# wenbowen123/iros20-6d-pose-tracking

Measured on NVIDIA H100. Metric: rgbd_pair_frames_per_sec, higher is better.
Workload: dtype bf16x3 (bf16 hi/lo split operands, 3 products/MAC, fp32 accumulate)

## Files before the change

iros20-6d-pose-tracking_b200/csrc/aux_kernels.cu:

```cuda
#include "aux_kernels.h"
#include "conv_common.h"
#include "bbox.cuh"
#include "launch.h"
#include "ptx.cuh"
#include "storage.cuh"
#include <cfloat>

namespace se3tn {


__device__ __forceinline__ float norm_f32(float x, float m, float s) { return __fdiv_rn(__fsub_rn(x, m), s); }
__device__ __forceinline__ float norm_f64(float x, double m, double s) { return static_cast<float>(__ddiv_rn(__dsub_rn(static_cast<double>(x), m), s)); }

__device__ __forceinline__ float depth_offset(unsigned d, double z1000, bool gl) {
    if (d <= 100u || d >= 2000u) return 2000.f;
    return static_cast<float>(gl ? __dadd_rn(static_cast<double>(d), z1000) : __dsub_rn(static_cast<double>(d), z1000));
}

constexpr int kPreRowsMax = 88;
constexpr int kDepthLo = 101, kDepthN = 1899;

template <int THREADS>
__global__ void __launch_bounds__(THREADS, THREADS == 256 ? 4 : 1)
preprocess_kernel(PreprocessArgs a, int rows_per_cta)
// ... 728 lines not shown
    if ((threadIdx.x & 31) == 0) atomicMax(amax_bits + blockIdx.y, __float_as_uint(m));
}
cudaError_t launch_amax_bf16x3(const AmaxArgs& a, unsigned* amax_bits, cudaStream_t s) {
    if (a.n_tensors <= 0 || a.n_tensors > AmaxArgs::kMax || a.n <= 0) return cudaErrorInvalidValue;
    for (int i = 0; i < a.n_tensors; ++i) if (a.t[i].nc % 4 || a.t[i].c0 % 4) return cudaErrorInvalidValue;
    amax_bf16x3_kernel<<<dim3(132, a.n_tensors), 256, 0, s>>>(a, amax_bits);
    return cudaGetLastError();
}

__global__ void split_stack_weights_kernel(const float* __restrict__ src, uint8_t* __restrict__ dst)
{
    const int i = blockIdx.x * blockDim.x + threadIdx.x;
    if (i >= 64 * 144) return;
    const int co = i / 144, k = (i - co * 144) * 4;
    const float* w = src + co * 576 + k;
    const float v[4] = {w[0], w[1], w[2], w[3]};
    const auto x = Storage<SE3TN_PREC_BF16X3>::encode(v);
    using B = Storage<SE3TN_PREC_BF16>;
    *reinterpret_cast<uint2*>(dst + B::addr(co, 576, k)) = x.get(0);
    *reinterpret_cast<uint2*>(dst + B::addr(64 + co, 576, k)) = x.get(1);
}
__global__ void split_stem_stack_kernel(const float* __restrict__ src, uint8_t* __restrict__ dst)
{
    const int i = blockIdx.x * blockDim.x + threadIdx.x;
    if (i >= 64 * 7 * 8) return;
    const int p = i & 7, r = (i >> 3) % 7, co = i / 56;
    const float* w = src + co * 224 + r * 32 + p * 4;
    const float v[4] = {w[0], w[1], w[2], w[3]};
    const auto x = Storage<SE3TN_PREC_BF16X3>::encode(v);
    const uint2 h = x.get(0), l = x.get(1);
    *reinterpret_cast<uint4*>(dst + (static_cast<size_t>(co) * 224 + r * 32 + p * 4) * 4) = make_uint4(h.x, h.y, h.x, h.y);
    *reinterpret_cast<uint4*>(dst + (static_cast<size_t>(64 + co) * 224 + r * 32 + p * 4) * 4) = make_uint4(l.x, l.y, 0u, 0u);
}
__global__ void permute_rows64_kernel(const float* __restrict__ src, float* __restrict__ dst, int ktot)
{
    const int i = blockIdx.x * blockDim.x + threadIdx.x;
    if (i >= 64 * ktot) return;
    const int col = i / ktot, k = i - col * ktot;
    const int ch = (col & 32) | (((col >> 1) & 3) << 3) | (((col >> 3) & 3) << 1) | (col & 1);
    dst[i] = src[ch * ktot + k];
}
cudaError_t launch_permute_rows64(const float* src, float* dst, int ktot, cudaStream_t s) {
    permute_rows64_kernel<<<(64 * ktot + 255) / 256, 256, 0, s>>>(src, dst, ktot);
    return cudaGetLastError();
}
cudaError_t launch_split_stack_weights(const float* src, void* dst, bool stem, cudaStream_t s) {
    if (stem) split_stem_stack_kernel<<<(64 * 7 * 8 + 127) / 128, 128, 0, s>>>(src, static_cast<uint8_t*>(dst));
    else split_stack_weights_kernel<<<(64 * 144 + 255) / 256, 256, 0, s>>>(src, static_cast<uint8_t*>(dst));
    return cudaGetLastError();
}

__global__ void pose_update_kernel(const double* poses_in, const float* __restrict__ trans,
                                   const float* __restrict__ rot, float tn, float rn,
                                   double* poses_out , int n)
{
    ptx::grid_dep_launch();
    ptx::grid_dep_wait();
    const int i = blockIdx.x * blockDim.x + threadIdx.x;
    if (i >= n) return;
    const float tr[3] = {trans[i * 3 + 0], trans[i * 3 + 1], trans[i * 3 + 2]};
    const float ro[3] = {rot[i * 3 + 0], rot[i * 3 + 1], rot[i * 3 + 2]};
    pose_update_one(poses_in + i * 16, tr, ro, tn, rn, poses_out + i * 16);
}

cudaError_t launch_pose_update(const double* poses_in, const float* trans, const float* rot, float tn, float rn,
                               double* poses_out, int n, cudaStream_t s) {
    if (n <= 0) return cudaSuccess;
    return launch_kernel(pose_update_kernel, dim3((n + 31) / 32), dim3(32), 0, s, true, poses_in, trans, rot, tn, rn, poses_out, n);
}

__device__ __forceinline__ void inv_transpose3(const double* m, double* o) {
    const double c00 = m[4] * m[8] - m[5] * m[7], c01 = m[5] * m[6] - m[3] * m[8], c02 = m[3] * m[7] - m[4] * m[6];
    const double det = m[0] * c00 + m[1] * c01 + m[2] * c02;
    const double id = 1.0 / det;
    o[0] = c00 * id; o[1] = c01 * id; o[2] = c02 * id;
    o[3] = (m[2] * m[7] - m[1] * m[8]) * id; o[4] = (m[0] * m[8] - m[2] * m[6]) * id; o[5] = (m[1] * m[6] - m[0] * m[7]) * id;
// ... 66 lines not shown
```

iros20-6d-pose-tracking_b200/csrc/aux_kernels.h:

```cpp
#pragma once
#include <cstdint>
#include <cuda_runtime.h>

namespace se3tn {

constexpr int kImg = 176;
constexpr int kStemH = kImg + 6;
constexpr int kStemW = kImg + 8;
constexpr size_t kStemImgFloats = static_cast<size_t>(kStemH) * kStemW * 4;

struct PreprocessArgs {
    const uint8_t* frame_rgb;
    const uint16_t* frame_depth;
    int H, W;
    double fx, fy, cx, cy;
    const double* poses;
    const double* object_width;
    const uint8_t* rgbA;
    const uint16_t* depthA;
    const int* weight_ids;
    const float* mean32; const float* std32;
    const double* mean64; const double* std64;
    int stats_f64;
    int stats_rows;
// ... 21 lines not shown
cudaError_t launch_crop_seg(const uint8_t* frame_rgb, const uint16_t* frame_depth, const uint8_t* seg, int H, int W, const int* bbox,
                            const int* class_ids, int n, int out_h, int out_w, uint8_t* crop_rgb, uint16_t* crop_depth,
                            uint8_t* crop_seg, int* count, cudaStream_t s);
struct AppendArgs {
    const uint8_t* rgbA; const uint16_t* depthA; const uint8_t* rgbB; const uint16_t* depthB;
    const int* count; const double* A_in_cam; const double* B_in_cam; const int* queue_ids;
    int n, num_queues, cap, min_count;
    int* tails;
    unsigned* done;
    uint8_t* q_rgbA; uint16_t* q_depthA; uint8_t* q_rgbB; uint16_t* q_depthB; double* q_A; double* q_B;
};
cudaError_t launch_append_pairs(const AppendArgs& a, cudaStream_t s);
cudaError_t launch_nchw_to_stem(const float* src, float* dst, int n, int precision, cudaStream_t s);
cudaError_t launch_maxpool(const float* in, float* out, int n_img, int Hin, int Win, int C, cudaStream_t s);
cudaError_t launch_head_pooled(const float* part , const float* fcw, const float* fcb, float* out_trans, float* out_rot,
                               int n_img, int npix, const int* img_wid, const float* const* fc_table,
                               const double* poses_in, double* poses_out, float tn, float rn, const LossArgs& loss,
                               unsigned* zero_words, int n_zero, cudaStream_t s);
cudaError_t launch_loss_reduce(const float* sq, int n, float* sums, cudaStream_t s);
cudaError_t launch_pair_loss(const float* trans, const float* rot, const double* trans_label, const double* rot_label,
                             const LossArgs& loss, int n, float* sums, cudaStream_t s);
cudaError_t launch_head(const float* x, const float* fcw, const float* fcb, float* out_trans, float* out_rot,
                        int n_img, int npix, cudaStream_t s);
cudaError_t launch_nhwc_to_nchw(const void* in, float* out, int n_img, int HW, int C, int precision, cudaStream_t s,
                                const float* fp8_scale = nullptr);
cudaError_t launch_encode_weights(int precision, const float* src, void* dst, int rows, int ktot, cudaStream_t s);
cudaError_t launch_encode_weights_fp8(const float* src, void* dst, float* row_scale, int rows, int ktot, cudaStream_t s);
struct AmaxArgs {
    static constexpr int kMax = 8;
    struct Tensor { const uint8_t* buf; int pixels, C, c0, nc; } t[kMax];
    int n_tensors, n;
};
cudaError_t launch_amax_bf16x3(const AmaxArgs& a, unsigned* amax_bits, cudaStream_t s);
cudaError_t launch_permute_rows64(const float* src , float* dst, int ktot, cudaStream_t s);
cudaError_t launch_split_stack_weights(const float* src, void* dst , bool stem, cudaStream_t s);
cudaError_t launch_pose_update(const double* poses_in, const float* trans, const float* rot, float tn, float rn,
                               double* poses_out, int n, cudaStream_t s);
cudaError_t launch_so3_log(const double* poses_a, const double* poses_b, double tn, double rn,
                           double* trans_label, double* rot_label, int n, cudaStream_t s);

}
```

iros20-6d-pose-tracking_b200/csrc/conv_common.h:

```cpp
#pragma once
#include <cstdint>
#include <cuda.h>
#include <cuda_runtime.h>

namespace se3tn {

constexpr int kMaxTaps = 9;
constexpr int kBlockM = 128;
constexpr int kChunkBytes = 128;

enum Act : int { ACT_NONE = 0, ACT_RELU = 1, ACT_SELU = 2 };
enum { KIND_S1 = 0, KIND_S2 = 1, KIND_STEM = 2 };

struct Tap {
    int16_t dy, dx;
};

struct ConvGeom {
    int Hin, Win, in_cstride, in_coff;
    int Ho, Wo, stride;
    int cin;
    int cout;
    int groups;
    int num_taps;
    int n_img;
    Tap taps[kMaxTaps];
    int out_cstride, out_coff;
    int res_cstride, res_coff;
    int act;
};

struct ConvPtrs {
    const float* in;
    const float* w;
    const float* bias;
    const float* res;
    float* out;
};

constexpr int kLayersPerSet = 14;
constexpr int kPoolSlices = 8;

struct LayerDesc {
    CUtensorMap amap[4];
    CUtensorMap bmap;
// ... 73 lines not shown
```

iros20-6d-pose-tracking_b200/csrc/conv_wgmma.cu:

```cuda
#include "conv_common.h"
#include "launch.h"
#include "ptx.cuh"
#include "storage.cuh"
#include <algorithm>

namespace se3tn {
namespace {

constexpr int kThreads2 = 384;
constexpr int kPoolPitch = 68;
constexpr int kPoolStageBytes = 121 * kPoolPitch * 4;
constexpr int kPoolStageAlloc = (kPoolStageBytes + 1023) & ~1023;
constexpr int kWgRowBytes = 64 * kChunkBytes;

template <int KIND> struct KTab;
template <> struct KTab<KIND_S1> {
    static constexpr int NU = 3;
    static constexpr int kAUnit = 19 * 1024;
    __host__ __device__ static constexpr int ntaps(int) { return 3; }
    __host__ __device__ static constexpr int wtap(int u, int k) { return k * 3 + u; }
    __host__ __device__ static constexpr int amap(int) { return 0; }
    __host__ __device__ static constexpr int c1(int u) { return u - 1; }
    __host__ __device__ static constexpr int c2(int) { return -1; }
    __host__ __device__ static constexpr int rows(int) { return 11 * 13; }
// ... 422 lines not shown
                    float4 mx = make_float4(-3.0e38f, -3.0e38f, -3.0e38f, -3.0e38f);
#pragma unroll
                    for (int dy = 0; dy < 3; ++dy)
#pragma unroll
                        for (int dx = 0; dx < 3; ++dx) {
                            const float4 s4 = *reinterpret_cast<const float4*>(stage + ((2 * ppy + dy) * 11 + 2 * ppx + dx) * kPoolPitch + c4);
                            mx.x = fmaxf(mx.x, s4.x); mx.y = fmaxf(mx.y, s4.y); mx.z = fmaxf(mx.z, s4.z); mx.w = fmaxf(mx.w, s4.w);
                        }
                    const float v4[4] = {selu_fast(mx.x + pb4.x), selu_fast(mx.y + pb4.y), selu_fast(mx.z + pb4.z), selu_fast(mx.w + pb4.w)};
                    S::encode(v4).store(L.out + S::addr((static_cast<size_t>(n0) * L.Ho + oy) * L.Wo + ox, L.out_c, L.out_coff + c4));
                }
                if constexpr (kShareStage) stage_turn.pass();
                else if constexpr (!PP) { if (C::kPoolBufs == 1) ptx::bar_sync(kEpiBar, 256); }
            }
            if (tstamp) tile_stamp(p.tile_trace, tile, 3);
        }
        if constexpr (PP) {
            turn.end(it);
            if constexpr (kShareStage) stage_turn.end(it);
        }
        if (stamp) { trace_stamp(p.trace, 4); trace_stamp(p.trace, 6); }
    }

    __syncthreads();
    if (threadIdx.x == 0) trace_exit(p.trace);
}

template <int PREC> struct TCfg {
    static constexpr int BN = 128;
    static constexpr int kAcc = BN / 2;
    static constexpr int kAStages = 3;
    static constexpr int kBStages = 6;
    static constexpr int kBTile = BN * kChunkBytes;
    static constexpr int kEpiPitch = 36;
    static constexpr int kEpiWarpBytes = 16 * kEpiPitch * 4 + 128;
    static constexpr int kEpiBytes = 8 * kEpiWarpBytes;
    static constexpr int kSched = 4;
    static constexpr int kAUnit = KTab<KIND_S1>::kAUnit;
    static_assert(kAUnit == KTab<KIND_S2>::kAUnit, "A ring stage size");
    static constexpr int kSmem = kAStages * kAUnit + kBStages * kBTile + ((kEpiBytes + 1023) & ~1023) + 1024 + 512;
    static_assert(kSmem <= 232448, "shared memory budget");
};
constexpr int kTaps3 = 9;

struct UnitCoord { int l, img, tx, ty, n_tile, grp, c0, c1, piece, gidx; };
__device__ __forceinline__ void unit_stamp(const TrunkParams& p, int u, int k) {
    if (p.trace && u < 2048) p.trace[256 * 8 + u * 5 + k] = k == 4 ? (gtimer() & ~0xffull) | (blockIdx.x & 0xff) : gtimer();
}

__device__ __forceinline__ int unit_layer(const TrunkParams& p, int u) {
    int l = 0;
#pragma unroll
    for (int i = 1; i < kTrunkMaxLayers; ++i) if (i < p.n_layers && u >= p.layer[i].unit_base) l = i;
    return l;
}

__device__ __forceinline__ UnitCoord decode_unit(const TrunkParams& p, int u) {
    UnitCoord c;
    c.l = unit_layer(p, u);
    const LayerDesc& L = p.layer[c.l];
    int local = u - L.unit_base;
    c.piece = 0; c.c0 = 0; c.c1 = L.chunks;
    if (p.ksplit > 1) {
        c.piece = local % p.ksplit; local /= p.ksplit;
        c.c0 = c.piece * L.chunks / p.ksplit; c.c1 = (c.piece + 1) * L.chunks / p.ksplit;
    }
    c.gidx = L.base_unit0 + local;
    const int im = local / L.units_per_image;
    int r = local - im * L.units_per_image;
    c.img = p.img_first + im;
    c.n_tile = r % L.n_tiles; r /= L.n_tiles;
    c.grp = r % L.groups; r /= L.groups;
    c.ty = r / L.tiles_x; c.tx = r - c.ty * L.tiles_x;
    return c;
}

template <int KIND, int PREC>
__device__ __forceinline__ void trunk_load_weights(const LayerDesc& L, const CUtensorMap* bm, const UnitCoord& c, uint8_t* sB,
                                                   uint64_t* b_full, uint64_t* b_empty, Ring<TCfg<PREC>::kBStages>& ring)
{
    using KT = KTab<KIND>;
    using C = TCfg<PREC>;
    const int wrow = c.grp * L.cout + c.n_tile * C::BN;
    for (int ch = c.c0; ch < c.c1; ++ch) {
#pragma unroll
        for (int u = 0; u < KT::NU; ++u) {
#pragma unroll
            for (int k = 0; k < KT::ntaps(u); ++k) {
                ptx::mbar_wait(&b_empty[ring.stage], ring.producer_parity());
                ptx::mbar_arrive_expect_tx(&b_full[ring.stage], C::kBTile);
                ptx::tma_load_2d(sB + ring.stage * C::kBTile, bm, &b_full[ring.stage], KT::wtap(u, k) * L.cin_words + ch * 32, wrow);
                ring.next();
            }
        }
    }
}

template <int KIND, int PREC>
__device__ __forceinline__ void trunk_mma_unit(float (&acc)[2][TCfg<PREC>::kAcc], const Consumer& cs, const Turn& turn, int chunks,
                                               uint8_t* sA, uint8_t* sB, uint64_t* a_full, uint64_t* a_empty, uint64_t* b_full,
                                               uint64_t* b_empty, Ring<TCfg<PREC>::kAStages>& a_ring, Ring<TCfg<PREC>::kBStages>& b_ring,
                                               unsigned long long* trace, bool first_unit, unsigned long long* ustamp)
{
    using KT = KTab<KIND>;
    using C = TCfg<PREC>;
    const bool stamp = cs.leader();
    uint32_t fresh = 0;
    int pend_b = -1, pend_a = -1;
    turn.wait();
    for (int ch = 0; ch < chunks; ++ch) {
#pragma unroll
        for (int u = 0; u < KT::NU; ++u) {
            ptx::mbar_wait(&a_full[a_ring.stage], a_ring.consumer_parity());
            if (first_unit && ch == 0 && u == 0 && stamp) trace_stamp(trace, 3);
            if (ustamp && ch == 0 && u == 0 && stamp) *ustamp = gtimer();
            const uint32_t a_unit_lo = desc_lo(sA + a_ring.stage * C::kAUnit);
#pragma unroll
            for (int k = 0; k < KT::ntaps(u); ++k) {
                ptx::mbar_wait(&b_full[b_ring.stage], b_ring.consumer_parity());
                if (first_unit && ch == 0 && u == 0 && k == 0 && stamp) trace_stamp(trace, 2);
                const uint32_t b_lo = desc_lo(sB + b_ring.stage * C::kBTile);
                ptx::wgmma_fence();
#pragma unroll
                for (int hf = 0; hf < 2; ++hf) {
                    const uint32_t a_lo = a_unit_lo + hf * (kWgRowBytes >> 4) + k * kRowShift * (kChunkBytes >> 4);
                    if constexpr (PREC == SE3TN_PREC_BF16X3) {
                        constexpr int AO[6] = {0, 2, 4, 6, 0, 2};
                        constexpr int BO[6] = {0, 2, 0, 2, 4, 6};
#pragma unroll
                        for (int i = 0; i < 6; ++i)
                            ptx::wgmma_bf16_n128(acc[hf], mk_desc(a_lo + AO[i]), mk_desc(b_lo + BO[i]), fresh | (i ? 1u : 0u));
                    } else {
                        mma_chunk<PREC, C::BN>(acc[hf], a_lo, b_lo, fresh);
                    }
                }
                ptx::wgmma_commit();
                ptx::wgmma_wait<1>();
                if (cs.leader()) {
                    if (pend_b >= 0) ptx::mbar_arrive(&b_empty[pend_b]);
                    if (pend_a >= 0) ptx::mbar_arrive(&a_empty[pend_a]);
                }
                pend_b = b_ring.stage;
                pend_a = (k + 1 == KT::ntaps(u)) ? a_ring.stage : -1;
                fresh = 1u;
                b_ring.next();
            }
            a_ring.next();
        }
    }
    turn.pass();
    ptx::wgmma_wait<0>();
    ptx::wgmma_reg_fence(acc[0]);
    ptx::wgmma_reg_fence(acc[1]);
    if (cs.leader()) {
        if (pend_b >= 0) ptx::mbar_arrive(&b_empty[pend_b]);
        if (pend_a >= 0) ptx::mbar_arrive(&a_empty[pend_a]);
    }
}

template <int PREC>
__global__ void __launch_bounds__(kThreads2, 1)
conv_trunk_kernel(const __grid_constant__ TrunkParams p)
{
    using C = TCfg<PREC>;
    constexpr int BN = C::BN;
    extern __shared__ uint8_t smem_raw[];
    uint8_t* smem = reinterpret_cast<uint8_t*>((reinterpret_cast<uintptr_t>(smem_raw) + 1023) & ~uintptr_t(1023));
    uint8_t* sA = smem;
    uint8_t* sB = sA + C::kAStages * C::kAUnit;
    uint8_t* sT = sB + C::kBStages * C::kBTile;
    uint64_t* bars = reinterpret_cast<uint64_t*>(sT + ((C::kEpiBytes + 1023) & ~1023));
    uint64_t* a_full = bars;
    uint64_t* a_empty = a_full + C::kAStages;
    uint64_t* b_full = a_empty + C::kAStages;
    uint64_t* b_empty = b_full + C::kBStages;
    uint64_t* sched_full = b_empty + C::kBStages;
    uint64_t* sched_empty = sched_full + C::kSched;
    int* sched_slot = reinterpret_cast<int*>(sched_empty + C::kSched);

    ptx::grid_dep_launch();
    if (threadIdx.x == 0) trace_stamp(p.trace, 0);
    const int warp = threadIdx.x >> 5;
    const int lane = threadIdx.x & 31;
    unsigned* done = p.sched + 1;

    if (threadIdx.x == 0) {
        for (int s = 0; s < C::kAStages; ++s) { ptx::mbar_init(&a_full[s], 1); ptx::mbar_init(&a_empty[s], 1); }
        for (int s = 0; s < C::kBStages; ++s) { ptx::mbar_init(&b_full[s], 1); ptx::mbar_init(&b_empty[s], 1); }
        for (int s = 0; s < C::kSched; ++s) { ptx::mbar_init(&sched_full[s], 1); ptx::mbar_init(&sched_empty[s], 9); }
        ptx::fence_barrier_init();
        ptx::fence_proxy_async();
    }
    __syncthreads();
    if (threadIdx.x == 0) trace_stamp(p.trace, 1);

    Ring<C::kSched> sring;
    auto next_unit = [&](bool whole_warp) -> int {
        ptx::mbar_wait(&sched_full[sring.stage], sring.consumer_parity());
        int u = 0;
        if (lane == 0) u = sched_slot[sring.stage];
        if (whole_warp) u = __shfl_sync(0xffffffffu, u, 0);
        if (lane == 0) ptx::mbar_arrive(&sched_empty[sring.stage]);
        sring.next();
        return u;
// ... 24 lines not shown
                            const long long t0 = clock64();
                            while (static_cast<unsigned>(ptx::ld_acquire_gpu(flag)) < L.dep_target) {
                                __nanosleep(64);
                                if (clock64() - t0 > (1ll << 34)) ptx::timeout_trap();
                            }
                        }
                        ptx::fence_proxy_async_all();
                    }
                    unit_stamp(p, u, 0);
                    const int cbase = c.grp * L.in_gstride_words;
                    if (L.kind == KIND_S1) load_a_units<KIND_S1>(L, c.tx * 11, c.ty * 11, cbase, c.img, c.c0, c.c1, sA, a_full, a_empty, a_ring);
                    else                   load_a_units<KIND_S2>(L, c.tx * 11, c.ty * 11, cbase, c.img, c.c0, c.c1, sA, a_full, a_empty, a_ring);
                    u = dealt ? u + static_cast<int>(gridDim.x) : static_cast<int>(atomicAdd(p.sched, 1u));
                }
            }
        } else if (warp == 1) {
            if (lane == 0) {
                if (!p.img_wid) for (int l = 0; l < p.n_layers; ++l) ptx::prefetch_tmap(&p.layer[l].bmap);
                Ring<C::kBStages> b_ring;
                for (;;) {
                    const int u = next_unit(false);
                    if (u >= p.total_units) break;
                    const UnitCoord c = decode_unit(p, u);
                    const LayerDesc& L = p.layer[c.l];
                    const CUtensorMap* bm = p.img_wid ? p.gbmaps + p.img_wid[c.img] * kLayersPerSet + L.li : &L.bmap;
                    if (L.kind == KIND_S1) trunk_load_weights<KIND_S1, PREC>(L, bm, c, sB, b_full, b_empty, b_ring);
                    else                   trunk_load_weights<KIND_S2, PREC>(L, bm, c, sB, b_full, b_empty, b_ring);
                }
            }
        }
    } else {
        ptx::setmaxnreg_inc<kConsumerRegs>();
        using S = Storage<PREC>;
        using R4 = Raw<PREC, 4>;
        ptx::grid_dep_wait();
        const Consumer cs;
        const int cw = cs.cw;
        float (*stg)[C::kEpiPitch] = reinterpret_cast<float (*)[C::kEpiPitch]>(sT + cs.ew * C::kEpiWarpBytes);
        int* rowtab = reinterpret_cast<int*>(sT + cs.ew * C::kEpiWarpBytes + 16 * C::kEpiPitch * 4);
        const int grp = lane & 7, sub = lane >> 3;
        Ring<C::kAStages> a_ring;
        Ring<C::kBStages> b_ring;
        const Turn turn{kTurnBar, cs.cg};
        turn.begin();
        for (int it = 0;; ++it) {
            const int u = next_unit(true);
            const bool mine = turn.mine(it);
            if (u >= p.total_units) { turn.end(it); break; }
            const UnitCoord c = decode_unit(p, u);
            const LayerDesc& L = p.layer[c.l];
            const int chunks = L.chunks / p.ksplit;
            if (!mine) {
                a_ring.skip(chunks * (L.kind == KIND_S1 ? KTab<KIND_S1>::NU : KTab<KIND_S2>::NU));
                b_ring.skip(chunks * kTaps3);
                continue;
            }
            {
                const int rw = 64 * (lane >> 4) + 16 * cw + (lane & 15);
                const int py = rw / 11, px = rw - py * 11;
                const int y = c.ty * 11 + py, x = c.tx * 11 + px;
                const bool valid = (rw < 121) && (y < L.Ho) && (x < L.Wo);
                __syncwarp();
                rowtab[lane] = valid ? (c.img * L.Ho + y) * L.Wo + x : -1;
                __syncwarp();
            }
            const int ch0 = c.grp * L.cout + c.n_tile * BN;
            const float* bias_base = p.img_wid ? p.gbias[p.img_wid[c.img] * kLayersPerSet + L.li] : L.bias;
            float4 b4[BN / 32];
#pragma unroll
            for (int bi = 0; bi < BN / 32; ++bi) b4[bi] = __ldg(reinterpret_cast<const float4*>(bias_base + ch0 + 32 * bi + grp * 4));
            const float* q8 = nullptr;
            float s_res = 1.f, inv_out = 1.f;
            if constexpr (PREC == SE3TN_PREC_FP8) {
                q8 = p.img_wid ? p.gfp8[p.img_wid[c.img]] : p.fp8;
                const int qg = L.q_grp_ch ? ch0 / L.q_grp_ch : 0;
                if (L.q_res >= 0) s_res = __ldg(q8 + L.q_res + qg);
                if (L.q_out >= 0) inv_out = 1.f / __ldg(q8 + L.q_out + qg);
            }

            float acc[2][C::kAcc];
#pragma unroll
            for (int i = 0; i < C::kAcc; ++i) { acc[0][i] = 0.f; acc[1][i] = 0.f; }
            unsigned long long* ust = (p.trace && u < 2048) ? p.trace + 256 * 8 + u * 5 + 1 : nullptr;
            if (L.kind == KIND_S1) trunk_mma_unit<KIND_S1, PREC>(acc, cs, turn, chunks, sA, sB, a_full, a_empty, b_full, b_empty, a_ring, b_ring, p.trace, it == 0, ust);
            else                   trunk_mma_unit<KIND_S2, PREC>(acc, cs, turn, chunks, sA, sB, a_full, a_empty, b_full, b_empty, a_ring, b_ring, p.trace, it == 0, ust);
            if (cs.leader()) { unit_stamp(p, u, 2); unit_stamp(p, u, 3); if (it == 0) trace_stamp(p.trace, 5); }
            int pix[2][4];
#pragma unroll
            for (int hf = 0; hf < 2; ++hf)
#pragma unroll
                for (int k = 0; k < 4; ++k) pix[hf][k] = rowtab[16 * hf + 4 * k + sub];

            if (L.res && L.dep_layer >= 0) {
                if (lane == 0) (void)ptx::ld_acquire_gpu(reinterpret_cast<const int*>(done + L.dep_layer * p.max_batch + c.img));
                __syncwarp();
            }
            const bool split = p.ksplit > 1;
            auto slice_of = [&](int pc) -> float* {
                return p.partial + ((static_cast<size_t>(c.gidx) * p.ksplit + pc) * 4 + cw) * (32 * BN);
            };
            unsigned own = 0xFu;
            if (split) {
                float4* d4 = reinterpret_cast<float4*>(slice_of(c.piece)) + lane;
#pragma unroll
                for (int hf = 0; hf < 2; ++hf)
#pragma unroll
                    for (int q = 0; q < C::kAcc / 4; ++q)
                        d4[(hf * C::kAcc / 4 + q) * 32] = make_float4(acc[hf][4 * q], acc[hf][4 * q + 1], acc[hf][4 * q + 2], acc[hf][4 * q + 3]);
                __threadfence();
                __syncwarp();
                if (lane == 0) atomicAdd(p.slice_cnt + c.gidx * 4 + cw, 1u);
                own = 0u;
#pragma unroll
                for (int bi = 0; bi < BN / 32; ++bi)
                    if (bi * p.ksplit / (BN / 32) == c.piece) own |= 1u << bi;
                if (lane == 0) {
                    const int* cnt = reinterpret_cast<const int*>(p.slice_cnt + c.gidx * 4 + cw);
                    const long long t0 = clock64();
                    while (ptx::ld_acquire_gpu(cnt) < p.ksplit) {
                        __nanosleep(32);
                        if (clock64() - t0 > (1ll << 34)) ptx::timeout_trap();
                    }
                }
                __syncwarp();
                __threadfence();
#pragma unroll
                for (int hf = 0; hf < 2; ++hf)
#pragma unroll
                    for (int bi = 0; bi < BN / 32; ++bi) {
                        if (!((own >> bi) & 1u)) continue;
#pragma unroll
                        for (int jj = 0; jj < 4; ++jj) {
                            float4 v[kSplitK];
#pragma unroll
                            for (int pc = 0; pc < kSplitK; ++pc)
                                if (pc < p.ksplit) v[pc] = __ldcg(reinterpret_cast<const float4*>(slice_of(pc)) + lane + (hf * C::kAcc / 4 + 4 * bi + jj) * 32);
                            float4 a = make_float4(0.f, 0.f, 0.f, 0.f);
#pragma unroll
                            for (int pc = 0; pc < kSplitK; ++pc)
                                if (pc < p.ksplit) { a.x += v[pc].x; a.y += v[pc].y; a.z += v[pc].z; a.w += v[pc].w; }
                            acc[hf][16 * bi + 4 * jj] = a.x; acc[hf][16 * bi + 4 * jj + 1] = a.y; acc[hf][16 * bi + 4 * jj + 2] = a.z; acc[hf][16 * bi + 4 * jj + 3] = a.w;
                        }
                    }
            }
#pragma unroll
            for (int hf = 0; hf < 2; ++hf) {
                const int slice = 4 * hf + cw;
#pragma unroll
                for (int bi = 0; bi < BN / 32; ++bi) {
                    if (!((own >> bi) & 1u)) continue;
                    const int chan = ch0 + 32 * bi;
                    R4 rr[4];
                    if (L.res) {
#pragma unroll
                        for (int k = 0; k < 4; ++k) {
                            rr[k] = R4{};
                            if (pix[hf][k] >= 0) {
                                const uint8_t* rp = L.res + S::addr(pix[hf][k], L.res_c, chan + grp * 4);
#pragma unroll
                                for (int q = 0; q < R4::kPieces; ++q) rr[k].set(q, __ldcg(R4::at(rp, q)));
                            }
                        }
                    }
                    __syncwarp();
#pragma unroll
                    for (int jj = 0; jj < 4; ++jj)
#pragma unroll
                        for (int h = 0; h < 2; ++h)
                            *reinterpret_cast<float2*>(&stg[cs.R + 8 * h][8 * jj + 2 * cs.m]) = make_float2(acc[hf][16 * bi + 4 * jj + 2 * h], acc[hf][16 * bi + 4 * jj + 2 * h + 1]);
                    float4 m4 = make_float4(1.f, 1.f, 1.f, 1.f);
                    if constexpr (PREC == SE3TN_PREC_FP8) m4 = __ldg(reinterpret_cast<const float4*>(q8 + L.fp8_mul + chan + grp * 4));
                    __syncwarp();
                    float4 a4[4];
#pragma unroll
                    for (int k = 0; k < 4; ++k) {
                        a4[k] = *reinterpret_cast<const float4*>(&stg[4 * k + sub][grp * 4]);
                        if constexpr (PREC == SE3TN_PREC_FP8) {
                            a4[k].x = a4[k].x * m4.x + b4[bi].x; a4[k].y = a4[k].y * m4.y + b4[bi].y;
                            a4[k].z = a4[k].z * m4.z + b4[bi].z; a4[k].w = a4[k].w * m4.w + b4[bi].w;
                        } else {
                            a4[k].x += b4[bi].x; a4[k].y += b4[bi].y; a4[k].z += b4[bi].z; a4[k].w += b4[bi].w;
                        }
                    }
                    if (L.res) {
#pragma unroll
                        for (int k = 0; k < 4; ++k) {
                            float r[4];
                            S::decode(rr[k], r);
                            if constexpr (PREC == SE3TN_PREC_FP8) { r[0] *= s_res; r[1] *= s_res; r[2] *= s_res; r[3] *= s_res; }
                            a4[k].x += r[0]; a4[k].y += r[1]; a4[k].z += r[2]; a4[k].w += r[3];
                        }
                    }
                    float4 psum = make_float4(0.f, 0.f, 0.f, 0.f);
#pragma unroll
                    for (int k = 0; k < 4; ++k) {
                        float4 o = a4[k];
                        o.x = act_apply(o.x, L.act); o.y = act_apply(o.y, L.act); o.z = act_apply(o.z, L.act); o.w = act_apply(o.w, L.act);
                        if (pix[hf][k] < 0) continue;
                        if (L.pool_part) { psum.x += o.x; psum.y += o.y; psum.z += o.z; psum.w += o.w; continue; }
                        if constexpr (PREC == SE3TN_PREC_FP8) { o.x *= inv_out; o.y *= inv_out; o.z *= inv_out; o.w *= inv_out; }
                        const float o4[4] = {o.x, o.y, o.z, o.w};
                        S::encode(o4).store(L.out + S::addr(pix[hf][k], L.out_c, L.out_coff + chan + grp * 4));
                    }
                    if (L.pool_part) {
#pragma unroll
                        for (int off = 8; off <= 16; off <<= 1) {
                            psum.x += __shfl_xor_sync(0xffffffffu, psum.x, off); psum.y += __shfl_xor_sync(0xffffffffu, psum.y, off);
                            psum.z += __shfl_xor_sync(0xffffffffu, psum.z, off); psum.w += __shfl_xor_sync(0xffffffffu, psum.w, off);
                        }
                        if (sub == 0)
                            *reinterpret_cast<float4*>(L.pool_part + (static_cast<size_t>(c.img) * kPoolSlices + slice) * L.out_c + L.out_coff + chan + grp * 4) = psum;
                    }
                }
            }
            if (c.l + 1 < p.n_layers) {
                ptx::fence_proxy_async_all();
                __threadfence();
                __syncwarp();
                if (lane == 0) atomicAdd(done + c.l * p.max_batch + c.img, 1u);
            }
            if (cs.leader()) unit_stamp(p, u, 4);
        }
        if (threadIdx.x == 128) { trace_stamp(p.trace, 4); trace_stamp(p.trace, 6); }
    }

    __syncthreads();
    if (threadIdx.x == 0) trace_exit(p.trace);
}

template <int KIND, int PREC>
cudaError_t launch_resident_t(const ResidentParams& p, int num_sms, bool pdl, cudaStream_t stream) {
    using C = RCfg<KIND, resident_prec(PREC)>;
    if (PREC == SE3TN_PREC_FP8 && ((!p.fp8 && !p.gfp8) || p.L.q_out < 0)) return cudaErrorInvalidValue;
    const int tiles_per_tap = (C::kStack == 2) ? 1 : p.L.chunks;
    if ((KIND == KIND_STEM ? 7 : 9) * tiles_per_tap > C::kMaxWTiles) return cudaErrorInvalidValue;
    if (C::kStack == 2 && KIND == KIND_S1 && p.L.chunks != 2) return cudaErrorInvalidValue;
    if (p.L.cout != 64 || p.L.groups != 1 || p.L.n_tiles != 1 || p.m_tiles <= 0) return cudaErrorInvalidValue;
    const bool pp = p.m_tiles > num_sms;
    const cudaError_t e = pp ? set_max_dynamic_smem<conv_resident_kernel<KIND, PREC, true>>(C::kSmem)
                             : set_max_dynamic_smem<conv_resident_kernel<KIND, PREC, false>>(C::kSmem);
    if (e != cudaSuccess) return e;
    return launch_kernel(pp ? conv_resident_kernel<KIND, PREC, true> : conv_resident_kernel<KIND, PREC, false>,
                         dim3(std::min(p.m_tiles, num_sms)), dim3(kThreads2), C::kSmem, stream, pdl, p);
}

template <int PREC>
// ... 52 lines not shown
```

iros20-6d-pose-tracking_b200/csrc/se3tn.cu:

```cuda
#include "../../include/se3tn.h"
#include "conv_common.h"
#include "aux_kernels.h"
#include "metrics.h"
#include "overlay.h"
#include "render.h"
#include <dlfcn.h>
#include "depth_fill.h"
#include "storage.cuh"

#include <algorithm>
#include <cmath>
#include <cstdio>
#include <cstdlib>
#include <cstring>
#include <map>
#include <memory>
#include <string>
#include <type_traits>
#include <vector>

using namespace se3tn;

namespace {

// ... 572 lines not shown
}

int queue_preprocess(se3tn_ctx* c, PreprocessArgs a, int n, cudaStream_t s) {
    a.mean32 = c->d_mean32.get(); a.std32 = c->d_std32.get(); a.mean64 = c->d_mean64.get(); a.std64 = c->d_std64.get();
    a.stats_f64 = c->stats_f64; a.stats_rows = c->stats_rows;
    a.stemA = c->buf[B_X0A]; a.stemB = c->buf[B_X0B];
    { ProfScope ps(c, 17, s); CU_TRY(c, launch_preprocess(a, n, s)); }
    ++c->launches;
    return SE3TN_OK;
}

int queue_render(se3tn_ctx* c, const double* K, const double* poses, const double* object_width, const int32_t* mesh_ids, int n,
                 int mode, int H, int W, uint8_t* rgbA, uint16_t* depthA, cudaStream_t s) {
    RenderArgs a;
    a.poses = poses; a.object_width = object_width; a.mesh_ids = mesh_ids; a.meshes = c->d_meshes.get(); a.n_meshes = c->mesh_rows;
    a.fx = K[0]; a.fy = K[1]; a.cx = K[2]; a.cy = K[3];
    a.rgb = rgbA; a.depth = depthA;
    a.mode = mode == SE3TN_RENDER_PYRENDER ? 1 : 0; a.vw = W; a.vh = H;
    a.projected = c->render_proj.get(); a.uniforms = c->render_unif.get(); a.max_nv = c->render_max_nv;
    { ProfScope ps(c, 20, s); CU_TRY(c, launch_render(a, n, s)); }
    c->launches += 2;
    return SE3TN_OK;
}

int prepare_weights(se3tn_ctx* c, DeviceWeights& w, const float* blob) {
    const size_t floats = blob_floats();
    CU_TRY(c, dev_alloc(w.blob, floats));
    for (int p : kTensorPrecs) CU_TRY(c, dev_alloc(w.conv[p], floats * prec_bytes_per_channel(p)));
    CU_TRY(c, dev_alloc(w.conv[SE3TN_PREC_FP8], floats));
    CU_TRY(c, dev_alloc(w.fp8, kFp8BlockFloats));
    CU_TRY(c, dev_alloc(w.fp8_sw, kFp8WRows));
    CU_TRY(c, dev_alloc(w.stack, 8 * 128 * 288 * sizeof(float)));
    CU_TRY(c, dev_alloc(w.perm, 6 * 64 * 576));
    DevBuf<float> perm_tmp;
    CU_TRY(c, dev_alloc(perm_tmp, 64 * 576));
    CU_TRY(c, cudaDeviceSynchronize());
    CU_TRY(c, cudaMemcpy(w.blob.get(), blob, floats * sizeof(float), cudaMemcpyHostToDevice));
    size_t off = 0;
    for (int li = 0; li < 14; ++li) {
        const LayerSpec& L = kLayers[li];
        const int rows = layer_rows(L), ktot = layer_ktot(L);
        w.w_off[li] = off; off += static_cast<size_t>(rows) * ktot;
        w.b_off[li] = off; off += rows;
        const float* wsrc = w.blob.get() + w.w_off[li];
        auto conv_dst = [&](int p) { return w.conv[p].get() + w.w_off[li] * prec_bytes_per_channel(p); };
        char what[64];
        int rc = SE3TN_OK;
        if (li >= kFirstTrunkLayer) {
            snprintf(what, sizeof what, "layer %d weights", li);
            for (int p : kTensorPrecs) {
                CU_TRY(c, launch_encode_weights(p, wsrc, conv_dst(p), rows, ktot, 0));
                if (!rc) rc = make_map2(c, &w.bmap[p][li], conv_dst(p), ktot * prec_bytes_per_channel(p) / 4, rows, L.block_n, what);
            }
            int sw_off = 0;
            for (int l = 0; l < li - kFirstTrunkLayer; ++l) sw_off += kFp8TrunkRows[l];
            CU_TRY(c, launch_encode_weights_fp8(wsrc, conv_dst(SE3TN_PREC_FP8), w.fp8_sw.get() + sw_off, rows, ktot, 0));
            if (!rc) rc = make_map2(c, &w.bmap[SE3TN_PREC_FP8][li], conv_dst(SE3TN_PREC_FP8), ktot / 4, rows, L.block_n, what);
        } else {
            const bool stem = (L.kind == K_STEM);
            void* w_tf32 = conv_dst(SE3TN_PREC_TF32);
            if (!stem) {
                if (ktot != 576 || rows != 64) return fail(c, SE3TN_ERR_STATE, "resident layer shape");
                CU_TRY(c, launch_permute_rows64(wsrc, perm_tmp.get(), 576, 0));
                wsrc = perm_tmp.get(); w_tf32 = w.perm.get() + static_cast<size_t>(li - 2) * 64 * 576;
            }
            snprintf(what, sizeof what, "layer %d resident weights", li);
            CU_TRY(c, launch_encode_weights(SE3TN_PREC_TF32, wsrc, w_tf32, 64, ktot, 0));
            rc = make_map2(c, &w.bmap[SE3TN_PREC_TF32][li], w_tf32, ktot, 64, 64, what);
            uint8_t* sdst = w.stack.get() + static_cast<size_t>(li) * 128 * 288 * sizeof(float);
            CU_TRY(c, launch_split_stack_weights(wsrc, sdst, stem, 0));
            if (!rc) rc = make_map2(c, &w.bmap[SE3TN_PREC_BF16X3][li], sdst, stem ? 224 : 288, 128, 128, what);
            for (int p : {SE3TN_PREC_BF16, SE3TN_PREC_FP16}) {
                if (stem) w.bmap[p][li] = w.bmap[stem_input_prec(p)][li];
                else {
                    CU_TRY(c, launch_encode_weights(p, wsrc, conv_dst(p), 64, ktot, 0));
                    if (!rc) rc = make_map2(c, &w.bmap[p][li], conv_dst(p), 288, 64, 64, what);
                }
            }
            w.bmap[SE3TN_PREC_FP8][li] = w.bmap[resident_prec(SE3TN_PREC_FP8)][li];
        }
        if (rc) return rc;
    }
    w.fc_off = off;
    CU_TRY(c, cudaDeviceSynchronize());
    w.fp8_sw_host.resize(kFp8WRows);
    CU_TRY(c, cudaMemcpy(w.fp8_sw_host.data(), w.fp8_sw.get(), kFp8WRows * sizeof(float), cudaMemcpyDeviceToHost));
    CU_TRY(c, cudaMemset(w.fp8.get(), 0, kFp8BlockFloats * sizeof(float)));
    CU_TRY(c, cudaDeviceSynchronize());
    return SE3TN_OK;
}

int upload_fp8(se3tn_ctx* c, WeightSet& ws, const float* scales) {
    const DeviceWeights& w = *ws.dev;
    std::vector<float> blk(kFp8BlockFloats, 0.f);
    for (int i = 0; i < SE3TN_FP8_SCALES; ++i) blk[i] = scales[i];
    int sw = 0;
    for (int l = 0; l < kTrunkMaxLayers; ++l) {
        float* mul = blk.data() + fp8_mul_off(l);
        for (int co = 0; co < kFp8TrunkRows[l]; ++co)
            mul[co] = scales[kFp8In[l] + (fp8_in_grouped(l) ? co / kFp8HeadCh : 0)] * w.fp8_sw_host[sw + co];
        sw += kFp8TrunkRows[l];
    }
    CU_TRY(c, cudaDeviceSynchronize());
    CU_TRY(c, cudaMemcpy(w.fp8.get(), blk.data(), blk.size() * sizeof(float), cudaMemcpyHostToDevice));
    memcpy(ws.fp8_scales, scales, sizeof ws.fp8_scales);
    ws.has_fp8 = true;
    return SE3TN_OK;
}

bool fp16_weights_fit(const float* blob) {
    size_t off = 0;
    for (const LayerSpec& L : kLayers) {
        const size_t nw = static_cast<size_t>(layer_rows(L)) * layer_ktot(L);
        if (L.kind != K_STEM)
            for (size_t i = 0; i < nw; ++i)
                if (std::fabs(blob[off + i]) > kFp16Max) return false;
        off += nw + layer_rows(L);
    }
    return true;
// ... 1121 lines not shown
```

Measured before the change: 35990.

## Permute trunk weight rows to match MMA fragments and drop smem epilogue staging

Trunk-layer weight rows are permuted at load time so each thread's wgmma accumulator fragment holds 8 contiguous output channels. The epilogue can then apply bias, residual, activation and the store straight from registers. This removes the shared-memory staging buffer, its warp syncs and the row table, and pooled sums are reduced with shuffles instead. Residual loads are prefetched one block ahead. The risk is correctness if the row permutation and the fp8 per-row scale remapping are inconsistent, plus higher register pressure. Trace stamps are also narrowed to 32 bits.

```diff
diff --git a/iros20-6d-pose-tracking_b200/csrc/aux_kernels.cu b/iros20-6d-pose-tracking_b200/csrc/aux_kernels.cu
--- a/iros20-6d-pose-tracking_b200/csrc/aux_kernels.cu
+++ b/iros20-6d-pose-tracking_b200/csrc/aux_kernels.cu
@@ -784,16 +784,16 @@
     *reinterpret_cast<uint4*>(dst + (static_cast<size_t>(co) * 224 + r * 32 + p * 4) * 4) = make_uint4(h.x, h.y, h.x, h.y);
     *reinterpret_cast<uint4*>(dst + (static_cast<size_t>(64 + co) * 224 + r * 32 + p * 4) * 4) = make_uint4(l.x, l.y, 0u, 0u);
 }
-__global__ void permute_rows64_kernel(const float* __restrict__ src, float* __restrict__ dst, int ktot)
+__global__ void permute_rows_kernel(const float* __restrict__ src, float* __restrict__ dst, int rows, int ktot)
 {
     const int i = blockIdx.x * blockDim.x + threadIdx.x;
-    if (i >= 64 * ktot) return;
+    if (i >= rows * ktot) return;
     const int col = i / ktot, k = i - col * ktot;
-    const int ch = (col & 32) | (((col >> 1) & 3) << 3) | (((col >> 3) & 3) << 1) | (col & 1);
-    dst[i] = src[ch * ktot + k];
-}
-cudaError_t launch_permute_rows64(const float* src, float* dst, int ktot, cudaStream_t s) {
-    permute_rows64_kernel<<<(64 * ktot + 255) / 256, 256, 0, s>>>(src, dst, ktot);
+    dst[i] = src[static_cast<size_t>(fragment_row_channel(col)) * ktot + k];
+}
+cudaError_t launch_permute_rows(const float* src, float* dst, int rows, int ktot, cudaStream_t s) {
+    if (rows % 32) return cudaErrorInvalidValue;
+    permute_rows_kernel<<<(rows * ktot + 255) / 256, 256, 0, s>>>(src, dst, rows, ktot);
     return cudaGetLastError();
 }
 cudaError_t launch_split_stack_weights(const float* src, void* dst, bool stem, cudaStream_t s) {
diff --git a/iros20-6d-pose-tracking_b200/csrc/aux_kernels.h b/iros20-6d-pose-tracking_b200/csrc/aux_kernels.h
--- a/iros20-6d-pose-tracking_b200/csrc/aux_kernels.h
+++ b/iros20-6d-pose-tracking_b200/csrc/aux_kernels.h
@@ -77,7 +77,7 @@
     int n_tensors, n;
 };
 cudaError_t launch_amax_bf16x3(const AmaxArgs& a, unsigned* amax_bits, cudaStream_t s);
-cudaError_t launch_permute_rows64(const float* src , float* dst, int ktot, cudaStream_t s);
+cudaError_t launch_permute_rows(const float* src , float* dst, int rows , int ktot, cudaStream_t s);
 cudaError_t launch_split_stack_weights(const float* src, void* dst , bool stem, cudaStream_t s);
 cudaError_t launch_pose_update(const double* poses_in, const float* trans, const float* rot, float tn, float rn,
                                double* poses_out, int n, cudaStream_t s);
diff --git a/iros20-6d-pose-tracking_b200/csrc/conv_common.h b/iros20-6d-pose-tracking_b200/csrc/conv_common.h
--- a/iros20-6d-pose-tracking_b200/csrc/conv_common.h
+++ b/iros20-6d-pose-tracking_b200/csrc/conv_common.h
@@ -11,6 +11,10 @@
 
 enum Act : int { ACT_NONE = 0, ACT_RELU = 1, ACT_SELU = 2 };
 enum { KIND_S1 = 0, KIND_S2 = 1, KIND_STEM = 2 };
+
+__host__ __device__ constexpr int fragment_row_channel(int row) {
+    return (row & ~31) | (((row >> 1) & 3) << 3) | (((row >> 3) & 3) << 1) | (row & 1);
+}
 
 struct Tap {
     int16_t dy, dx;
diff --git a/iros20-6d-pose-tracking_b200/csrc/conv_wgmma.cu b/iros20-6d-pose-tracking_b200/csrc/conv_wgmma.cu
--- a/iros20-6d-pose-tracking_b200/csrc/conv_wgmma.cu
+++ b/iros20-6d-pose-tracking_b200/csrc/conv_wgmma.cu
@@ -478,20 +478,21 @@
     static constexpr int kAStages = 3;
     static constexpr int kBStages = 6;
     static constexpr int kBTile = BN * kChunkBytes;
-    static constexpr int kEpiPitch = 36;
-    static constexpr int kEpiWarpBytes = 16 * kEpiPitch * 4 + 128;
-    static constexpr int kEpiBytes = 8 * kEpiWarpBytes;
     static constexpr int kSched = 4;
     static constexpr int kAUnit = KTab<KIND_S1>::kAUnit;
     static_assert(kAUnit == KTab<KIND_S2>::kAUnit, "A ring stage size");
-    static constexpr int kSmem = kAStages * kAUnit + kBStages * kBTile + ((kEpiBytes + 1023) & ~1023) + 1024 + 512;
+    static constexpr int kSmem = kAStages * kAUnit + kBStages * kBTile + 1024 + 512;
     static_assert(kSmem <= 232448, "shared memory budget");
 };
 constexpr int kTaps3 = 9;
 
 struct UnitCoord { int l, img, tx, ty, n_tile, grp, c0, c1, piece, gidx; };
+constexpr int kTraceUnits = 5 * 256 * 8 * 2 / 5;
+__device__ __forceinline__ unsigned* unit_stamps(const TrunkParams& p, int u) {
+    return (p.trace && u < kTraceUnits) ? reinterpret_cast<unsigned*>(p.trace + 256 * 8) + u * 5 : nullptr;
+}
 __device__ __forceinline__ void unit_stamp(const TrunkParams& p, int u, int k) {
-    if (p.trace && u < 2048) p.trace[256 * 8 + u * 5 + k] = k == 4 ? (gtimer() & ~0xffull) | (blockIdx.x & 0xff) : gtimer();
+    if (unsigned* s = unit_stamps(p, u)) s[k] = k == 4 ? (static_cast<unsigned>(gtimer()) & ~0xffu) | (blockIdx.x & 0xff) : static_cast<unsigned>(gtimer());
 }
 
 __device__ __forceinline__ int unit_layer(const TrunkParams& p, int u) {
@@ -546,7 +547,7 @@
 __device__ __forceinline__ void trunk_mma_unit(float (&acc)[2][TCfg<PREC>::kAcc], const Consumer& cs, const Turn& turn, int chunks,
                                                uint8_t* sA, uint8_t* sB, uint64_t* a_full, uint64_t* a_empty, uint64_t* b_full,
                                                uint64_t* b_empty, Ring<TCfg<PREC>::kAStages>& a_ring, Ring<TCfg<PREC>::kBStages>& b_ring,
-                                               unsigned long long* trace, bool first_unit, unsigned long long* ustamp)
+                                               unsigned long long* trace, bool first_unit, unsigned* ustamp)
 {
     using KT = KTab<KIND>;
     using C = TCfg<PREC>;
@@ -559,7 +560,7 @@
         for (int u = 0; u < KT::NU; ++u) {
             ptx::mbar_wait(&a_full[a_ring.stage], a_ring.consumer_parity());
             if (first_unit && ch == 0 && u == 0 && stamp) trace_stamp(trace, 3);
-            if (ustamp && ch == 0 && u == 0 && stamp) *ustamp = gtimer();
+            if (ustamp && ch == 0 && u == 0 && stamp) *ustamp = static_cast<unsigned>(gtimer());
             const uint32_t a_unit_lo = desc_lo(sA + a_ring.stage * C::kAUnit);
 #pragma unroll
             for (int k = 0; k < KT::ntaps(u); ++k) {
@@ -614,8 +615,7 @@
     uint8_t* smem = reinterpret_cast<uint8_t*>((reinterpret_cast<uintptr_t>(smem_raw) + 1023) & ~uintptr_t(1023));
     uint8_t* sA = smem;
     uint8_t* sB = sA + C::kAStages * C::kAUnit;
-    uint8_t* sT = sB + C::kBStages * C::kBTile;
-    uint64_t* bars = reinterpret_cast<uint64_t*>(sT + ((C::kEpiBytes + 1023) & ~1023));
+    uint64_t* bars = reinterpret_cast<uint64_t*>(sB + C::kBStages * C::kBTile);
     uint64_t* a_full = bars;
     uint64_t* a_empty = a_full + C::kAStages;
     uint64_t* b_full = a_empty + C::kAStages;
@@ -706,13 +706,10 @@
     } else {
         ptx::setmaxnreg_inc<kConsumerRegs>();
         using S = Storage<PREC>;
-        using R4 = Raw<PREC, 4>;
+        using R8 = Raw<PREC, 8>;
         ptx::grid_dep_wait();
         const Consumer cs;
         const int cw = cs.cw;
-        float (*stg)[C::kEpiPitch] = reinterpret_cast<float (*)[C::kEpiPitch]>(sT + cs.ew * C::kEpiWarpBytes);
-        int* rowtab = reinterpret_cast<int*>(sT + cs.ew * C::kEpiWarpBytes + 16 * C::kEpiPitch * 4);
-        const int grp = lane & 7, sub = lane >> 3;
         Ring<C::kAStages> a_ring;
         Ring<C::kBStages> b_ring;
         const Turn turn{kTurnBar, cs.cg};
@@ -729,20 +726,8 @@
                 b_ring.skip(chunks * kTaps3);
                 continue;
             }
-            {
-                const int rw = 64 * (lane >> 4) + 16 * cw + (lane & 15);
-                const int py = rw / 11, px = rw - py * 11;
-                const int y = c.ty * 11 + py, x = c.tx * 11 + px;
-                const bool valid = (rw < 121) && (y < L.Ho) && (x < L.Wo);
-                __syncwarp();
-                rowtab[lane] = valid ? (c.img * L.Ho + y) * L.Wo + x : -1;
-                __syncwarp();
-            }
             const int ch0 = c.grp * L.cout + c.n_tile * BN;
             const float* bias_base = p.img_wid ? p.gbias[p.img_wid[c.img] * kLayersPerSet + L.li] : L.bias;
-            float4 b4[BN / 32];
-#pragma unroll
-            for (int bi = 0; bi < BN / 32; ++bi) b4[bi] = __ldg(reinterpret_cast<const float4*>(bias_base + ch0 + 32 * bi + grp * 4));
             const float* q8 = nullptr;
             float s_res = 1.f, inv_out = 1.f;
             if constexpr (PREC == SE3TN_PREC_FP8) {
@@ -755,15 +740,21 @@
             float acc[2][C::kAcc];
 #pragma unroll
             for (int i = 0; i < C::kAcc; ++i) { acc[0][i] = 0.f; acc[1][i] = 0.f; }
-            unsigned long long* ust = (p.trace && u < 2048) ? p.trace + 256 * 8 + u * 5 + 1 : nullptr;
+            unsigned* ust = unit_stamps(p, u);
+            if (ust) ++ust;
             if (L.kind == KIND_S1) trunk_mma_unit<KIND_S1, PREC>(acc, cs, turn, chunks, sA, sB, a_full, a_empty, b_full, b_empty, a_ring, b_ring, p.trace, it == 0, ust);
             else                   trunk_mma_unit<KIND_S2, PREC>(acc, cs, turn, chunks, sA, sB, a_full, a_empty, b_full, b_empty, a_ring, b_ring, p.trace, it == 0, ust);
             if (cs.leader()) { unit_stamp(p, u, 2); unit_stamp(p, u, 3); if (it == 0) trace_stamp(p.trace, 5); }
-            int pix[2][4];
+            int pix[2][2];
 #pragma unroll
             for (int hf = 0; hf < 2; ++hf)
 #pragma unroll
-                for (int k = 0; k < 4; ++k) pix[hf][k] = rowtab[16 * hf + 4 * k + sub];
+                for (int h = 0; h < 2; ++h) {
+                    const int rw = cs.row(hf, h);
+                    const int py = rw / 11, px = rw - py * 11;
+                    const int y = c.ty * 11 + py, x = c.tx * 11 + px;
+                    pix[hf][h] = (rw < 121) && (y < L.Ho) && (x < L.Wo) ? (c.img * L.Ho + y) * L.Wo + x : -1;
+                }
 
             if (L.res && L.dep_layer >= 0) {
                 if (lane == 0) (void)ptx::ld_acquire_gpu(reinterpret_cast<const int*>(done + L.dep_layer * p.max_batch + c.img));
@@ -817,75 +808,97 @@
                         }
                     }
             }
-#pragma unroll
-            for (int hf = 0; hf < 2; ++hf) {
-                const int slice = 4 * hf + cw;
-#pragma unroll
-                for (int bi = 0; bi < BN / 32; ++bi) {
-                    if (!((own >> bi) & 1u)) continue;
-                    const int chan = ch0 + 32 * bi;
-                    R4 rr[4];
+            struct BlockRes { R8 res[2]; };
+            auto load_res = [&](int hf, int bi, BlockRes& a) {
+                const int chan = ch0 + 32 * bi + 8 * cs.m;
+#pragma unroll
+                for (int h = 0; h < 2; ++h) {
+                    a.res[h] = R8{};
+                    if (L.res && pix[hf][h] >= 0) {
+                        const uint8_t* rp = L.res + S::addr(pix[hf][h], L.res_c, chan);
+#pragma unroll
+                        for (int q = 0; q < R8::kPieces; ++q) a.res[h].set(q, __ldcg(R8::at(rp, q)));
+                    }
+                }
+            };
+            constexpr int kBlocks = 2 * BN / 32;
+            BlockRes cur, nxt;
+            if (own & 1u) load_res(0, 0, cur);
+#pragma unroll
+            for (int q = 0; q < kBlocks; ++q) {
+                const int hf = q >> 2, bi = q & 3;
+                if (q + 1 < kBlocks && ((own >> ((q + 1) & 3)) & 1u)) load_res((q + 1) >> 2, (q + 1) & 3, nxt);
+                if (!((own >> bi) & 1u)) { cur = nxt; continue; }
+                const int chan = ch0 + 32 * bi + 8 * cs.m;
+                const float4 bA = __ldg(reinterpret_cast<const float4*>(bias_base + chan)), bB = __ldg(reinterpret_cast<const float4*>(bias_base + chan + 4));
+                const float bias8[8] = {bA.x, bA.y, bA.z, bA.w, bB.x, bB.y, bB.z, bB.w};
+                float mul8[8] = {1.f, 1.f, 1.f, 1.f, 1.f, 1.f, 1.f, 1.f};
+                if constexpr (PREC == SE3TN_PREC_FP8) {
+                    const float4 mA = __ldg(reinterpret_cast<const float4*>(q8 + L.fp8_mul + chan));
+                    const float4 mB = __ldg(reinterpret_cast<const float4*>(q8 + L.fp8_mul + chan + 4));
+                    mul8[0] = mA.x; mul8[1] = mA.y; mul8[2] = mA.z; mul8[3] = mA.w; mul8[4] = mB.x; mul8[5] = mB.y; mul8[6] = mB.z; mul8[7] = mB.w;
+                }
+                float o[2][8];
+#pragma unroll
+                for (int h = 0; h < 2; ++h) {
+                    float* v = o[h];
+#pragma unroll
+                    for (int jj = 0; jj < 4; ++jj)
+#pragma unroll
+                        for (int e = 0; e < 2; ++e) {
+                            const float a = acc[hf][16 * bi + 4 * jj + 2 * h + e];
+                            if constexpr (PREC == SE3TN_PREC_FP8) v[2 * jj + e] = a * mul8[2 * jj + e] + bias8[2 * jj + e];
+                            else                                  v[2 * jj + e] = a + bias8[2 * jj + e];
+                        }
                     if (L.res) {
-#pragma unroll
-                        for (int k = 0; k < 4; ++k) {
-                            rr[k] = R4{};
-                            if (pix[hf][k] >= 0) {
-                                const uint8_t* rp = L.res + S::addr(pix[hf][k], L.res_c, chan + grp * 4);
-#pragma unroll
-                                for (int q = 0; q < R4::kPieces; ++q) rr[k].set(q, __ldcg(R4::at(rp, q)));
-                            }
+                        float r[8];
+                        S::decode(cur.res[h], r);
+#pragma unroll
+                        for (int e = 0; e < 8; ++e) {
+                            if constexpr (PREC == SE3TN_PREC_FP8) r[e] *= s_res;
+                            v[e] += r[e];
                         }
                     }
-                    __syncwarp();
-#pragma unroll
-                    for (int jj = 0; jj < 4; ++jj)
-#pragma unroll
-                        for (int h = 0; h < 2; ++h)
-                            *reinterpret_cast<float2*>(&stg[cs.R + 8 * h][8 * jj + 2 * cs.m]) = make_float2(acc[hf][16 * bi + 4 * jj + 2 * h], acc[hf][16 * bi + 4 * jj + 2 * h + 1]);
-                    float4 m4 = make_float4(1.f, 1.f, 1.f, 1.f);
-                    if constexpr (PREC == SE3TN_PREC_FP8) m4 = __ldg(reinterpret_cast<const float4*>(q8 + L.fp8_mul + chan + grp * 4));
-                    __syncwarp();
-                    float4 a4[4];
-#pragma unroll
-                    for (int k = 0; k < 4; ++k) {
-                        a4[k] = *reinterpret_cast<const float4*>(&stg[4 * k + sub][grp * 4]);
-                        if constexpr (PREC == SE3TN_PREC_FP8) {
-                            a4[k].x = a4[k].x * m4.x + b4[bi].x; a4[k].y = a4[k].y * m4.y + b4[bi].y;
-                            a4[k].z = a4[k].z * m4.z + b4[bi].z; a4[k].w = a4[k].w * m4.w + b4[bi].w;
-                        } else {
-                            a4[k].x += b4[bi].x; a4[k].y += b4[bi].y; a4[k].z += b4[bi].z; a4[k].w += b4[bi].w;
+                    if (L.act == ACT_SELU) {
+#pragma unroll
+                        for (int e = 0; e < 8; ++e) v[e] = selu_fast(v[e]);
+                    } else if (L.act == ACT_RELU) {
+#pragma unroll
+                        for (int e = 0; e < 8; ++e) v[e] = fmaxf(v[e], 0.f);
+                    }
+                    if (L.pool_part || pix[hf][h] < 0) continue;
+                    if constexpr (PREC == SE3TN_PREC_FP8) {
+#pragma unroll
+                        for (int e = 0; e < 8; ++e) v[e] *= inv_out;
+                    }
+                    S::encode(o[h]).store(L.out + S::addr(pix[hf][h], L.out_c, L.out_coff + chan));
+                }
+                if (L.pool_part) {
+                    const bool lo = cs.R < 4;
+                    float s[4];
+#pragma unroll
+                    for (int e = 0; e < 4; ++e) {
+                        float own_v[2], other[2];
+#pragma unroll
+                        for (int h = 0; h < 2; ++h) {
+                            const float mine = pix[hf][h] >= 0 ? (lo ? o[h][e] : o[h][4 + e]) : 0.f;
+                            const float give = pix[hf][h] >= 0 ? (lo ? o[h][4 + e] : o[h][e]) : 0.f;
+                            own_v[h] = mine;
+                            other[h] = __shfl_xor_sync(0xffffffffu, give, 16);
                         }
-                    }
-                    if (L.res) {
-#pragma unroll
-                        for (int k = 0; k < 4; ++k) {
-                            float r[4];
-                            S::decode(rr[k], r);
-                            if constexpr (PREC == SE3TN_PREC_FP8) { r[0] *= s_res; r[1] *= s_res; r[2] *= s_res; r[3] *= s_res; }
-                            a4[k].x += r[0]; a4[k].y += r[1]; a4[k].z += r[2]; a4[k].w += r[3];
-                        }
-                    }
-                    float4 psum = make_float4(0.f, 0.f, 0.f, 0.f);
-#pragma unroll
-                    for (int k = 0; k < 4; ++k) {
-                        float4 o = a4[k];
-                        o.x = act_apply(o.x, L.act); o.y = act_apply(o.y, L.act); o.z = act_apply(o.z, L.act); o.w = act_apply(o.w, L.act);
-                        if (pix[hf][k] < 0) continue;
-                        if (L.pool_part) { psum.x += o.x; psum.y += o.y; psum.z += o.z; psum.w += o.w; continue; }
-                        if constexpr (PREC == SE3TN_PREC_FP8) { o.x *= inv_out; o.y *= inv_out; o.z *= inv_out; o.w *= inv_out; }
-                        const float o4[4] = {o.x, o.y, o.z, o.w};
-                        S::encode(o4).store(L.out + S::addr(pix[hf][k], L.out_c, L.out_coff + chan + grp * 4));
-                    }
-                    if (L.pool_part) {
-#pragma unroll
-                        for (int off = 8; off <= 16; off <<= 1) {
-                            psum.x += __shfl_xor_sync(0xffffffffu, psum.x, off); psum.y += __shfl_xor_sync(0xffffffffu, psum.y, off);
-                            psum.z += __shfl_xor_sync(0xffffffffu, psum.z, off); psum.w += __shfl_xor_sync(0xffffffffu, psum.w, off);
-                        }
-                        if (sub == 0)
-                            *reinterpret_cast<float4*>(L.pool_part + (static_cast<size_t>(c.img) * kPoolSlices + slice) * L.out_c + L.out_coff + chan + grp * 4) = psum;
-                    }
-                }
+                        const float r0 = lo ? own_v[0] : other[0], r4 = lo ? other[0] : own_v[0];
+                        const float r8 = lo ? own_v[1] : other[1], r12 = lo ? other[1] : own_v[1];
+                        s[e] = (((0.f + r0) + r4) + r8) + r12;
+                    }
+#pragma unroll
+                    for (int off = 4; off <= 8; off <<= 1)
+#pragma unroll
+                        for (int e = 0; e < 4; ++e) s[e] += __shfl_xor_sync(0xffffffffu, s[e], off);
+                    if ((cs.R & 3) == 0)
+                        *reinterpret_cast<float4*>(L.pool_part + (static_cast<size_t>(c.img) * kPoolSlices + 4 * hf + cw) * L.out_c + L.out_coff +
+                                                   chan + (lo ? 0 : 4)) = make_float4(s[0], s[1], s[2], s[3]);
+                }
+                cur = nxt;
             }
             if (c.l + 1 < p.n_layers) {
                 ptx::fence_proxy_async_all();
diff --git a/iros20-6d-pose-tracking_b200/csrc/se3tn.cu b/iros20-6d-pose-tracking_b200/csrc/se3tn.cu
--- a/iros20-6d-pose-tracking_b200/csrc/se3tn.cu
+++ b/iros20-6d-pose-tracking_b200/csrc/se3tn.cu
@@ -628,8 +628,10 @@
     CU_TRY(c, dev_alloc(w.fp8_sw, kFp8WRows));
     CU_TRY(c, dev_alloc(w.stack, 8 * 128 * 288 * sizeof(float)));
     CU_TRY(c, dev_alloc(w.perm, 6 * 64 * 576));
+    size_t perm_floats = 0;
+    for (const LayerSpec& L : kLayers) perm_floats = std::max(perm_floats, static_cast<size_t>(layer_rows(L)) * layer_ktot(L));
     DevBuf<float> perm_tmp;
-    CU_TRY(c, dev_alloc(perm_tmp, 64 * 576));
+    CU_TRY(c, dev_alloc(perm_tmp, perm_floats));
     CU_TRY(c, cudaDeviceSynchronize());
     CU_TRY(c, cudaMemcpy(w.blob.get(), blob, floats * sizeof(float), cudaMemcpyHostToDevice));
     size_t off = 0;
@@ -644,6 +646,8 @@
         int rc = SE3TN_OK;
         if (li >= kFirstTrunkLayer) {
             snprintf(what, sizeof what, "layer %d weights", li);
+            CU_TRY(c, launch_permute_rows(wsrc, perm_tmp.get(), rows, ktot, 0));
+            wsrc = perm_tmp.get();
             for (int p : kTensorPrecs) {
                 CU_TRY(c, launch_encode_weights(p, wsrc, conv_dst(p), rows, ktot, 0));
                 if (!rc) rc = make_map2(c, &w.bmap[p][li], conv_dst(p), ktot * prec_bytes_per_channel(p) / 4, rows, L.block_n, what);
@@ -657,7 +661,7 @@
             void* w_tf32 = conv_dst(SE3TN_PREC_TF32);
             if (!stem) {
                 if (ktot != 576 || rows != 64) return fail(c, SE3TN_ERR_STATE, "resident layer shape");
-                CU_TRY(c, launch_permute_rows64(wsrc, perm_tmp.get(), 576, 0));
+                CU_TRY(c, launch_permute_rows(wsrc, perm_tmp.get(), 64, 576, 0));
                 wsrc = perm_tmp.get(); w_tf32 = w.perm.get() + static_cast<size_t>(li - 2) * 64 * 576;
             }
             snprintf(what, sizeof what, "layer %d resident weights", li);
@@ -679,8 +683,10 @@
     }
     w.fc_off = off;
     CU_TRY(c, cudaDeviceSynchronize());
+    std::vector<float> sw_rows(kFp8WRows);
+    CU_TRY(c, cudaMemcpy(sw_rows.data(), w.fp8_sw.get(), kFp8WRows * sizeof(float), cudaMemcpyDeviceToHost));
     w.fp8_sw_host.resize(kFp8WRows);
-    CU_TRY(c, cudaMemcpy(w.fp8_sw_host.data(), w.fp8_sw.get(), kFp8WRows * sizeof(float), cudaMemcpyDeviceToHost));
+    for (int co = 0; co < kFp8WRows; ++co) w.fp8_sw_host[co] = sw_rows[fragment_row_channel(co)];
     CU_TRY(c, cudaMemset(w.fp8.get(), 0, kFp8BlockFloats * sizeof(float)));
     CU_TRY(c, cudaDeviceSynchronize());
     return SE3TN_OK;
```

After: 36450, median of 6. +1.3%, better.
